# XiandaGuo/OpenStereo

Hardware: AMD Instinct MI355X
Metric: stereo-pairs/s at 540x960 D=192 (GwcNet fwd) (higher is better)
Workload: dtype f32 via f16x3 split-MFMA (hi/lo fp16 operands, f32 accumulate; HBM tensors f32); 1 GPU; GwcNet-gc inference, SceneFlow-shaped 540x960 padded to 544x960, D=192, G=40 + 12ch concat (BASELINE configs[1]); weights=deterministic synthetic (sharpened), random-init architecture, sub_batch_streams=3, parallelism=independent pairs x1, precision=f16x3, launch=hipGraph replay

## Files before the change

include/openstereo_amd.h:

```cpp
#ifndef OPENSTEREO_AMD_H
#define OPENSTEREO_AMD_H

#include <stddef.h>

#ifdef __cplusplus
extern "C" {
#endif

#define OSA_ABI_VERSION 17
#define OSA_META_FLOATS 128

enum { OSA_NCDHW = 0, OSA_NDHWC = 1 };
enum { OSA_ACT_NONE = 0, OSA_ACT_RELU = 1, OSA_ACT_LEAKY = 2, OSA_ACT_RELU6 = 3, OSA_ACT_SIGMOID = 4, OSA_ACT_TANH = 5 };
enum { OSA_GATE_RAW = 16 };
#define OSA_GATE_CHANNELS(n) ((int)((unsigned)(n) << 16))
enum { OSA_IN_SPLIT = 32, OSA_OUT_SPLIT = 64, OSA_RES_SPLIT = 128, OSA_REDIR_SPLIT = 256 };
enum { OSA_RES_AFTER_ACT = 512 };

int         osa_abi_version(void);
const char* osa_last_error(void);
const char* osa_target_arch(void);

int osa_build_volume_f32(const float* left_gwc, const float* right_gwc, int C, int num_groups,
                         const float* left_cat, const float* right_cat, int Cc,
                         float* vol, int layout, int vol_channels, int c_off,
                         int B, int H, int W, int maxdisp, int mask_left_concat,
                         float* vol_meta, void* stream);

int osa_build_volume_nhwc_f32(const float* left_gwc, const float* right_gwc, int C, int num_groups, int gwc_stride,
                              const float* left_cat, const float* right_cat, int Cc, int cat_stride,
                              float* vol, int vol_channels, int c_off,
                              int B, int H, int W, int maxdisp, int mask_left_concat, float* vol_meta, void* stream);
int osa_cat_fms_f32(const float* reference_fm, const float* target_fm, float* out, const int* disp_index,
                    int B, int C, int H, int W, int n_samples, void* stream);
int osa_pair_volume_f32(const float* left, const float* right, float* out,
                        int B, int C, int groups, int H, int W, int planes, int mode, void* stream);

int osa_corr_volume_f32(const float* left, const float* right, float* vol,
                        int B, int C, int H, int W, int maxdisp, void* stream);

int osa_ncdhw_to_ndhwc_f32(const float* x, float* y, int B, int C, long long S,
                           int yCs, int c_off, void* stream);
// ... 331 lines not shown
                            const float* mean3, const float* std3,
                            float* out, int layout, void* stream);

enum { OSA_IN_F16 = 32, OSA_OUT_F16 = 64, OSA_RES_F16 = 128 };
int osa_conv3d_pack_f16(const float* w_ref, float* w_packed, int Ci, int Co, int kd, int kh, int kw, void* stream);
int osa_deconv3d_pack_f16(const float* w_ref, float* w_packed, int Ci, int Co, int k, int pad, void* stream);
int osa_deconv2d_pack_f16(const float* w_ref, float* w_packed, int Ci, int Co, int k, int pad, void* stream);
int osa_conv3d_ndhwc_f16(const void* x, const float* w_packed, const float* scale, const float* shift, const void* residual, void* y,
                         int B, int Di, int Hi, int Wi, int Ci, int xCs, int Co, int yCs, int rCs, int kd, int kh, int kw, int stride,
                         int pad_d, int pad_h, int pad_w, int dil_d, int dil_h, int dil_w, const float* gate_logits, int gCs,
                         int act, float slope, void* stream);
int osa_deconv3d_ndhwc_f16(const void* x, const float* w_packed, const float* scale, const float* shift, const void* residual, void* y,
                           int B, int Di, int Hi, int Wi, int Ci, int xCs, int Co, int yCs, int rCs, int k, int pad, int opad,
                           const float* gate_logits, int gCs, int act, float slope, void* stream);
int osa_deconv2d_nhwc_f16(const void* x, const float* w_packed, const float* scale, const float* shift, const void* residual, void* y,
                          int B, int Hi, int Wi, int Ci, int xCs, int Co, int yCs, int rCs, int k, int pad, int opad,
                          const float* gate_logits, int gCs, int act, float slope, void* stream);

size_t osa_channel_sums_workspace_bytes(long long P, int C);
int osa_channel_sums(const void* dy, int dy_f16, int dy_cs, const void* x, int x_f16, int x_cs, const float* x_shift,
                     const float* dx_scale, void* dx, int dx_cs, long long P, int C,
                     float* out, float* workspace, size_t workspace_bytes, void* stream);
int osa_channel_sums_multi(const void* const* dys, int n_items, int dy_f16, int dy_cs, long long P, int C,
                           float* out, float* workspace, size_t workspace_bytes, void* stream);
int osa_channel_affine(const void* u, int u_f16, int u_cs, const void* v, int v_f16, int v_cs,
                       const float* a, const float* b, const float* c0, void* out, int out_cs,
                       long long P, int C, int relu, void* stream);

size_t osa_instnorm_workspace_floats(int B, long long HW, int C);
int osa_instnorm_nhwc_f32(const float* x, float* y, int B, long long HW, int C, int xCs, int yCs, float eps, int act, float slope,
                          float* workspace, float* y_meta, void* stream);

long long osa_conv3d_march_launches(void);

long long osa_conv3d_march_s2_launches(void);
int osa_conv_march_s2_segment_planes(int planes);

int osa_deconv_walk(int enable);
int osa_deconv_walk_segment_planes(int planes);
long long osa_deconv3d_walk_launches(void);

int osa_conv_b_ring_mask(int mask);
long long osa_conv_b_ring_launches(void);

int osa_volume_walk_step(int step);
long long osa_volume_walk_launches(void);

int osa_build_volume_nhwc_split_eligible(const float* left_cat, const float* right_cat, const float* vol, int C, int num_groups,
                                         int gwc_stride, int Cc, int cat_stride, int vol_channels, int c_off, int W, int maxdisp);
int osa_build_volume_nhwc_split_f16x3(const float* left_gwc, const float* right_gwc, int C, int num_groups, int gwc_stride,
                                      const float* left_cat, const float* right_cat, int Cc, int cat_stride,
                                      float* vol, int vol_channels, int c_off,
                                      int B, int H, int W, int maxdisp, int mask_left_concat,
                                      const float* gwc_meta, const float* cat_meta, float* vol_meta, void* stream);

#ifdef __cplusplus
}
#endif
#endif
```

openstereo_amd/_lib.py:

```python
from __future__ import annotations

import ctypes as C
import os
import threading

_HERE = os.path.dirname(os.path.abspath(__file__))
LIB_PATH = os.environ.get("OSA_LIB_PATH") or os.path.join(_HERE, "lib", "libopenstereo_amd.so")

_lock = threading.Lock()
_lib = None

c_fp = C.c_void_p
c_i = C.c_int
c_f = C.c_float
c_st = C.c_void_p
c_ll = C.c_longlong


class F16x3Ranges(C.Structure):
    _fields_ = [("x_meta", C.c_void_p), ("residual_meta", C.c_void_p), ("redir_meta", C.c_void_p),
                ("y_meta", C.c_void_p), ("bound_coef", C.c_void_p), ("redir_bound_coef", C.c_void_p), ("weight_scale", C.c_void_p)]


c_rng = C.POINTER(F16x3Ranges)
# ... 43 lines not shown
    **dict.fromkeys(("osa_deconv2d_nhwc_f32", "osa_deconv2d_nhwc_f16"), (c_i, [c_fp] * 6 + [c_i] * 11 + [c_fp, c_i, c_i, c_f, c_st])),
    "osa_deconv2d_nhwc_f16x3": (c_i, [c_fp] * 6 + [c_i] * 11 + [c_fp, c_i, c_i, c_f, c_f, c_rng, c_st]),
    "osa_dwconv2d_pack_f32": (c_i, [c_fp, c_fp, c_i, c_i, c_i, c_st]),
    "osa_dwconv2d_nhwc_f32": (c_i, [c_fp] * 6 + [c_i] * 15 + [c_fp, c_st]),
    "osa_dwconv2d_nhwc_f16io": (c_i, [c_fp, c_i, c_fp, c_fp, c_fp, c_fp, c_i] + [c_i] * 11 + [c_i, c_fp, c_st]),
    "osa_gru_combine_f32": (c_i, [c_fp, c_fp, c_fp, c_fp, c_ll, c_i, c_i, c_i, c_i, c_i, c_fp, c_st]),
    "osa_gru_gates_rz_fwd": (c_i, [c_ref, c_fp, c_fp, c_ref, c_ref, c_ref, c_ref, c_ref, c_ll, c_i, c_st]),
    "osa_gru_gates_rz_bwd": (c_i, [c_ref, c_fp, c_fp, c_ref, c_ref, c_ref, c_ref, c_ref, c_ref, c_ref, c_ll, c_i, c_st]),
    "osa_gru_gates_q_fwd": (c_i, [c_ref, c_ref, c_fp, c_ref, c_ref, c_ref, c_ll, c_i, c_st]),
    "osa_gru_gates_q_bwd": (c_i, [c_ref, c_ref, c_fp, c_ref, c_ref, c_ref, c_ref, c_ref, c_ref, c_ll, c_i, c_st]),
    "osa_disp_update_f32": (c_i, [c_fp, c_fp, c_i, c_fp, c_fp, c_i, c_ll, c_fp, c_fp, c_st]),
    "osa_conv3d_pack_ex_auto": (c_i, [c_fp, c_fp, c_i, c_i, c_i, c_i, c_i, c_i, c_i, c_fp, c_fp, c_st]),
    **dict.fromkeys(("osa_deconv3d_pack_f16x3_auto", "osa_deconv2d_pack_f16x3_auto"), (c_i, [c_fp, c_fp, c_i, c_i, c_i, c_i, c_fp, c_fp, c_st])),
    "osa_cat_fms_f32": (c_i, [c_fp, c_fp, c_fp, c_fp, c_i, c_i, c_i, c_i, c_i, c_st]),
    "osa_pool2x_nhwc_f32": (c_i, [c_fp, c_fp, c_i, c_i, c_i, c_i, c_i, c_i, c_fp, c_fp, c_st]),
    "osa_resize_bilinear_nhwc_f32": (c_i, [c_fp, c_fp, c_i, c_i, c_i, c_i, c_i, c_i, c_i, c_i, c_fp, c_fp, c_st]),
    "osa_context_upsample_logits_f32": (c_i, [c_fp, c_fp, c_i, C.POINTER(c_ll), c_fp, c_i, c_i, c_i, c_i, c_f, c_st]),
    "osa_context_upsample_logits_bwd_f32": (c_i, [c_fp, c_fp, c_i, C.POINTER(c_ll), c_fp, c_fp, c_fp, C.POINTER(c_ll), c_fp, c_i, c_i, c_i, c_i, c_f, c_st]),
    "osa_context_upsample_f32": (c_i, [c_fp, c_fp, c_fp, c_i, c_i, c_i, c_i, c_i, c_f, c_st]),
    "osa_geo_rows_f32": (c_i, [c_fp, c_fp, c_i, c_i, c_i, c_i, c_i, c_i, c_st]),
    "osa_avgpool_rows_f32": (c_i, [c_fp, c_fp, c_ll, c_i, c_st]),
    **dict.fromkeys(("osa_geo_lookup_f32", "osa_geo_lookup_bwd_acc_f32", "osa_geo_lookup_bwd_f32"), (c_i, _LEVELS + [c_fp, c_fp, c_fp, c_i, c_i, c_i, c_i, c_i, c_st])),
    "osa_geo_lookup_nhwc_f32": (c_i, _LEVELS + [c_fp, c_fp, c_fp, c_i, c_i, c_i, c_i, c_i, c_i, c_st]),
    **dict.fromkeys(("osa_geo_lookup_mr_f32", "osa_geo_lookup_mr_bwd_acc_f32"), (c_i, _LEVELS + [c_fp, c_i, c_fp, c_i, c_fp, c_fp, c_fp, c_fp, c_fp, c_fp, c_i, c_i, c_i, c_i, c_i, c_st])),
    "osa_geo_lookup_mr_nhwc_f32": (c_i, _LEVELS + [c_fp, c_i, c_fp, c_i, c_fp, c_fp, c_fp, c_fp, c_fp, c_fp, c_i, c_i, c_i, c_i, c_i, c_i, c_i, c_i, c_i, c_st]),
    "osa_preprocess_pair_f32": (c_i, [c_fp, c_fp, c_i, c_i, c_i, c_i, c_i, C.POINTER(c_f), C.POINTER(c_f), c_fp, c_i, c_st]),
    "osa_instnorm_workspace_floats": (C.c_size_t, [c_i, c_ll, c_i]),
    "osa_instnorm_nhwc_f32": (c_i, [c_fp, c_fp, c_i, c_ll, c_i, c_i, c_i, c_f, c_i, c_f, c_fp, c_fp, c_st]),
    "osa_conv3d_wgrad_ws_multi": (c_i, [c_i, c_fp, c_fp, c_i, c_fp] + [c_i] * 22 + [c_fp, c_fp, c_i, c_i, c_fp, C.c_size_t, c_st]),
    "osa_channel_sums_workspace_bytes": (C.c_size_t, [c_ll, c_i]),
    "osa_channel_affine": (c_i, [c_fp, c_i, c_i, c_fp, c_i, c_i, c_fp, c_fp, c_fp, c_fp, c_i, c_ll, c_i, c_i, c_st]),
    "osa_channel_sums_multi": (c_i, [c_fp, c_i, c_i, c_i, c_ll, c_i, c_fp, c_fp, C.c_size_t, c_st]),
    "osa_channel_sums": (c_i, [c_fp, c_i, c_i, c_fp, c_i, c_i, c_fp, c_fp, c_fp, c_i, c_ll, c_i, c_fp, c_fp, C.c_size_t, c_st]),
    **dict.fromkeys(("osa_conv3d_march_launches", "osa_conv3d_march_s2_launches", "osa_deconv3d_walk_launches", "osa_conv_b_ring_launches", "osa_volume_walk_launches"), (c_ll, [])),
    **dict.fromkeys(("osa_deconv_walk", "osa_deconv_walk_segment_planes", "osa_conv_march_s2_segment_planes", "osa_conv_b_ring_mask", "osa_volume_walk_step"), (c_i, [c_i])),
    "osa_build_volume_nhwc_split_eligible": (c_i, [c_fp, c_fp, c_fp, c_i, c_i, c_i, c_i, c_i, c_i, c_i, c_i, c_i]),
    "osa_build_volume_nhwc_split_f16x3": (c_i, [c_fp, c_fp, c_i, c_i, c_i, c_fp, c_fp, c_i, c_i, c_fp] + [c_i] * 7 + [c_fp, c_fp, c_fp, c_st]),
    "osa_upsample_softargmin_f32": (c_i, [c_fp, c_fp, c_i, c_i, c_i, c_i, c_i, c_i, c_i, c_i, c_st]),
    **dict.fromkeys(("osa_softargmin_var_f32", "osa_softmax_softargmin_var_bwd_f32"), (c_i, [c_fp, c_fp, c_fp, c_fp, c_i, c_i, c_i, c_i, c_st])),
    "osa_softargmin_var_bwd_f32": (c_i, [c_fp, c_fp, c_fp, c_fp, c_fp, c_fp, c_i, c_i, c_i, c_i, c_st]),
    "osa_upsample_softargmin_var_bwd_ws_f32": (c_i, [c_fp, c_fp, c_fp, c_fp, c_i, c_i, c_i, c_i, c_i, c_i, c_i, c_i, c_fp, C.c_size_t, c_st]),
    "osa_mr_volume_f32": (c_i, [c_fp] * 7 + [c_i] * 12 + [c_st]),
    "osa_mr_volume_bwd_ws_f32": (c_i, [c_fp] * 3 + [c_i] + [c_fp] * 8 + [c_i] * 11 + [c_fp, C.c_size_t, c_st]),
    **dict.fromkeys(("osa_mv2_block3d_packed_floats", "osa_mv2_block2d_packed_floats"), (C.c_size_t, [c_i] * 3)),
    **dict.fromkeys(("osa_mv2_block3d_pack_f32", "osa_mv2_block2d_pack_f32"), (c_i, [c_fp] * 10 + [c_i] * 3 + [c_st])),
    "osa_mv2_block3d_f32": (c_i, [c_fp] * 3 + [c_i] * 9 + [c_st]),
    **dict.fromkeys(("osa_mv2_block2d_f32", "osa_disparity_attention_f32"), (c_i, [c_fp] * 4 + [c_i] * 9 + [c_st])),
    "osa_disparity_attention_pack_f32": (c_i, [c_fp] * 8 + [c_i] * 4 + [c_st]),
    "osa_interlaced_volume_pack_f32": (c_i, [c_fp] * 13 + [c_i] * 4 + [c_st]),
    "osa_interlaced_volume_f32": (c_i, [c_fp] * 4 + [c_i] * 8 + [c_st]),
}


class EngineError(RuntimeError):
    pass


def load():
    global _lib
    if _lib is not None:
        return _lib
    with _lock:
        if _lib is not None:
            return _lib
        if not os.path.exists(LIB_PATH):
            raise EngineError(f"{LIB_PATH} is missing: build it with `python -m openstereo_amd.build` (hipcc, gfx950). There is no CPU fallback.")
        lib = C.CDLL(LIB_PATH)
        for name, (res, args) in SIGNATURES.items():
            fn = getattr(lib, name)
            fn.restype = res
            fn.argtypes = args
        if lib.osa_abi_version() != abi_version(lib):
            raise EngineError(f"ABI version mismatch: library reports {lib.osa_abi_version()}, include/openstereo_amd.h declares {abi_version(lib)}")
        if os.environ.get("OSA_B_RING_MASK"):
            lib.osa_conv_b_ring_mask(int(os.environ["OSA_B_RING_MASK"], 0))
        if os.environ.get("OSA_DECONV_WALK"):
            lib.osa_deconv_walk(int(os.environ["OSA_DECONV_WALK"], 0))
        if os.environ.get("OSA_VOL_WALK"):
            lib.osa_volume_walk_step(int(os.environ["OSA_VOL_WALK"]))
        _lib = lib
    return _lib


_abi = None


def abi_version(lib=None) -> int:
    global _abi
    if _abi is None:
        import re
        hdr = os.path.join(os.path.dirname(os.path.abspath(__file__)), "..", "include", "openstereo_amd.h")
        try:
            with open(hdr) as f:
                _abi = int(re.search(r"#define\s+OSA_ABI_VERSION\s+(\d+)", f.read()).group(1))
        except (OSError, AttributeError):
            h = lib if lib is not None else _lib
            if h is None:
                return -1
            _abi = int(h.osa_abi_version())
    return _abi


CALLS = {}


def call(name: str, *args):
    lib = load()
    CALLS[name] = CALLS.get(name, 0) + 1
    rc = getattr(lib, name)(*args)
    if rc != 0:
        msg = lib.osa_last_error()
        raise EngineError(f"{name} failed ({rc}): {msg.decode() if msg else '?'}")
# ... 2 lines not shown
```

openstereo_amd/csrc/conv_march.h:

```cpp
#pragma once
#include "conv_kernel.h"

namespace osa {

template <int NWV, int TW>
struct MarchGeo {
    static constexpr int MT = 2;
    static constexpr int RPT = 32 / TW;
    static constexpr int TH = NWV * MT * RPT;
    static constexpr int LH = TH + 2, LW = TW + 2;
    static constexpr int VQ = 5;
    static constexpr int ROWQ = (TW == 16) ? ((LW * VQ + 15) / 16 * 16) : LW * VQ;
    static constexpr int NPI = (LH * ROWQ + 63) / 64;
    static constexpr int PLANEQ = NPI * 64;
    static constexpr int NP = (NPI + NWV - 1) / NWV;
    static constexpr int NTHR = NWV * 64;
    static constexpr int BRING = 4;
    static constexpr int BSTEPQ = 6 * 64;
    static constexpr size_t lds_bytes() { return (size_t)2 * PLANEQ * 16 + (size_t)BRING * BSTEPQ * 16; }
    static_assert((size_t)NWV * 32 * 36 * 4 <= (size_t)PLANEQ * 16, "epilogue tiles must fit into one plane buffer");
    static_assert(NP <= 7, "one piece per wave and step, all of them forced home by the waits of steps 2..8");
};

template <int NWV, int TW, int OUTS, int INS>
__global__ __launch_bounds__(NWV * 64, 2) void conv_march_kernel(const ConvArgs p, const int dseg, const int nseg) {
    using G = MarchGeo<NWV, TW>;
    constexpr int MT = G::MT, TH = G::TH, ROWQ = G::ROWQ, VQ = G::VQ, PLANEQ = G::PLANEQ, NTHR = G::NTHR, NP = G::NP, NPI = G::NPI;
    extern __shared__ __attribute__((aligned(16))) float4 smem[];
    float4* const bring = smem + 2 * PLANEQ;

    const int tid = threadIdx.x, lane = tid & 63;
    const int wm = __builtin_amdgcn_readfirstlane(tid >> 6);
    const int col = lane & 31, hh = lane >> 5;

    unsigned bid = xcd_remap(blockIdx.x, gridDim.x);
    const int twi = bid % p.tilesW; bid /= p.tilesW;
    const int thi = bid % p.tilesH; bid /= p.tilesH;
    const int seg = bid % nseg;
    const int b = (int)(bid / nseg);
    const int d0 = seg * dseg, d1 = (d0 + dseg < p.Di) ? d0 + dseg : p.Di;
    const int a0h = thi * TH, a0w = twi * TW;
    const int g0h = a0h - 1, g0w = a0w - 1;

    float s_in = 1.f, s_res_inv = 1.f, s_out = 1.f;
    if (p.in_meta) s_in = INS ? p.in_meta[1] : pow2_scale(amax_read(p.in_meta));
    if (p.res && p.res_meta && (p.act & OSA_RES_SPLIT)) s_res_inv = 1.0f / p.res_meta[1];
    if (OUTS && p.coef && p.in_meta) {
        float bound = p.coef[0] * amax_read(p.in_meta) + p.coef[1];
        if (p.res && p.res_meta) bound += amax_read(p.res_meta);
        s_out = pow2_scale(bound * 1.0625f);
    }
    if (OUTS && p.out_meta && blockIdx.x == 0 && tid == 0) p.out_meta[1] = s_out;
    const float osc = (p.wscale_dev ? p.wscale_dev[1] : p.oscale) * (1.0f / s_in);
    float am = 0.f;
    unsigned amax_seen = 0u;
    if (p.out_meta) amax_seen = amax_peek(p.out_meta);

    int abase[MT];
#pragma unroll
    for (int m = 0; m < MT; ++m) {
        const int q = (wm * MT + m) * 32 + col;
        abase[m] = (q / TW) * ROWQ + (q % TW) * VQ + hh;
    }

    f32x16 acc[3][MT];
#pragma unroll
    for (int s = 0; s < 3; ++s)
#pragma unroll
        for (int m = 0; m < MT; ++m)
#pragma unroll
            for (int r = 0; r < 16; ++r) acc[s][m][r] = 0.f;

    const int bstep = 2 * p.CoP;
    const int tstep = 2 * bstep;
// ... 121 lines not shown
                            r = mul4(r, s_res_inv);
                        }
                        float o[4] = {fmaf(a.x, sc[h2].x, sh[h2].x) + r.x, fmaf(a.y, sc[h2].y, sh[h2].y) + r.y,
                                      fmaf(a.z, sc[h2].z, sh[h2].z) + r.z, fmaf(a.w, sc[h2].w, sh[h2].w) + r.w};
#pragma unroll
                        for (int e = 0; e < 4; ++e) o[e] = (o[e] < 0.f) ? (act_relu ? 0.f : o[e] * act_ns) : o[e];
                        if (ok) am = fmaxf(am, fmaxf(fmaxf(fabsf(o[0]), fabsf(o[1])), fmaxf(fabsf(o[2]), fabsf(o[3]))));
                        split_f16(make_float4(o[0] * s_out, o[1] * s_out, o[2] * s_out, o[3] * s_out), hq[h2], lq[h2]);
                    }
                    if (ok) {
                        float* ys = yb + vox * p.yCs + soff;
                        store16(ys, make_uint4(hq[0].x, hq[0].y, hq[1].x, hq[1].y));
                        store16(ys + 8, make_uint4(lq[0].x, lq[0].y, lq[1].x, lq[1].y));
                    }
                }
            }
        }
    };


    const int pf = (d0 - 1 > 0) ? d0 - 1 : 0, pl = (d1 < p.Di - 1) ? d1 : p.Di - 1;
    const int npass = (pl - pf + 1) * nch;
    if constexpr (INS) {
#pragma unroll
        for (int i = 0; i < NP; ++i) dma_piece(i, 0, pf, 0);
    }
    dma_b(0, 0, 0); dma_b(1, 0, 1); dma_b(2, 0, 2);

    int pd = pf, c = 0;
    for (int q = 0; q < npass; ++q) {
        const int cn = (c + 1 < nch) ? c + 1 : 0;
        const int pdn = (q + 1 < npass) ? ((c + 1 < nch) ? pd : pd + 1) : -1;
        const int sb = q & 3, cur = q & 1;
        if constexpr (!INS) {
            __syncthreads();
            stage_brick<NTHR, PREC_F16X3, 1, 4>(p, smem + cur * PLANEQ, PLANEQ, b, c * CC, pd, g0h, g0w, tid, s_in);
        }
        if (!INS || q == 0) asm volatile("s_waitcnt vmcnt(0)" ::: "memory");
        __syncthreads();
        int ab[MT];
#pragma unroll
        for (int m = 0; m < MT; ++m) ab[m] = abase[m] + cur * PLANEQ;
        int bq[4];
#pragma unroll
        for (int k = 0; k < 4; ++k) bq[k] = (((sb + k) & 3) * 6) * 64 + lane;
        float4 A[2][MT][2], B[3][2];
        auto load_a = [&](float4 (&An)[MT][2], const int khw) {
            const int off = (khw / 3) * ROWQ + (khw % 3) * VQ;
#pragma unroll
            for (int m = 0; m < MT; ++m) { An[m][0] = smem[ab[m] + off]; An[m][1] = smem[ab[m] + off + 2]; }
        };
        auto load_b = [&](float4 (&Bn)[2], const int u) {
            const int kd = u % 3;
            Bn[0] = bring[bq[(u / 3) & 3] + (kd * 2) * 64]; Bn[1] = bring[bq[(u / 3) & 3] + (kd * 2 + 1) * 64];
        };
        load_b(B[0], 0);
        load_b(B[1], 1);
        load_a(A[0], 0);
#pragma unroll
        for (int s = 0; s < 9; ++s) {
            if (s > 0) { __builtin_amdgcn_s_barrier(); asm volatile("" ::: "memory"); }
            if (s + 3 < 9) dma_b((sb + s + 3) & 3, c, s + 3);
            else dma_b((sb + s + 3) & 3, cn, s + 3 - 9);
            if (s < NP) dma_piece(s, cur ^ 1, pdn, cn);
            if (s + 1 < 9) load_a(A[(s + 1) & 1], s + 1);
#pragma unroll
            for (int kd = 0; kd < 3; ++kd) {
                const int u = s * 3 + kd;
                if (u + 2 < 27) load_b(B[(u + 2) % 3], u + 2);
                __builtin_amdgcn_sched_barrier(0);
#pragma unroll
                for (int term = 0; term < 3; ++term)
#pragma unroll
                    for (int m = 0; m < MT; ++m) {
                        const f16x8 a = __builtin_bit_cast(f16x8, A[s & 1][m][term == 1 ? 1 : 0]);
                        const f16x8 w = __builtin_bit_cast(f16x8, B[u % 3][term == 0 ? 1 : 0]);
                        acc[2 - kd][m] = __builtin_amdgcn_mfma_f32_32x32x16_f16(a, w, acc[2 - kd][m], 0, 0, 0);
                    }
                __builtin_amdgcn_sched_barrier(0);
            }
            constexpr int PCS = INS ? 1 : 0;
            wait_vmcnt(NI + ((s < NP) ? PCS : 0) + ((s >= 1 && s - 1 < NP) ? PCS : 0));
        }
        if (c + 1 == nch) {
            const bool v2 = (pd - 1 >= d0) && (pd - 1 < d1);
            if (v2) {
                __syncthreads();
                epilogue(pd - 1, reinterpret_cast<float*>(smem + cur * PLANEQ) + wm * (32 * 36));
            }
#pragma unroll
            for (int m = 0; m < MT; ++m) {
                acc[0][m] = acc[1][m]; acc[1][m] = acc[2][m];
#pragma unroll
                for (int r = 0; r < 16; ++r) acc[2][m][r] = 0.f;
            }
            if (q + 1 == npass && pd + 1 == d1 && pd + 1 >= p.Di) {
                __syncthreads();
                epilogue(pd, reinterpret_cast<float*>(smem + cur * PLANEQ) + wm * (32 * 36));
            }
            ++pd; c = 0;
        } else ++c;
    }
    asm volatile("s_waitcnt vmcnt(0)" ::: "memory");
    if (p.out_meta) {
        __syncthreads();
        publish_amax(p.out_meta, am, amax_seen, reinterpret_cast<float*>(smem));
    }
}

}
```

openstereo_amd/csrc/conv_march.hip:

```cpp
#include "conv_march.h"
#include "conv_march_s2.h"
#include "conv_deconv_walk.h"

namespace osa {

static long long g_march_launches = 0;
long long march_launches() { return g_march_launches; }

struct MarchCfg { int nwv, tw, th; size_t lds; void (*fn[2][2])(const ConvArgs, int, int); };
#define OSA_MARCH_CFG(NWV, TW) { NWV, TW, MarchGeo<NWV, TW>::TH, MarchGeo<NWV, TW>::lds_bytes(),                      \
                                 { { conv_march_kernel<NWV, TW, 0, 0>, conv_march_kernel<NWV, TW, 0, 1> },            \
                                   { conv_march_kernel<NWV, TW, 1, 0>, conv_march_kernel<NWV, TW, 1, 1> } } }
static const MarchCfg g_march_cfgs[] = {
    OSA_MARCH_CFG(4, 16),
    OSA_MARCH_CFG(4, 32),
};

int launch_conv_march(ConvArgs& a, hipStream_t st, const char* what) {
    if (!exp_int("OSA_MARCH", 1)) return 0;
    if (a.T != 27 || a.Co != 32 || a.CoP != 32 || a.Di < 3 || a.gate || a.rx) return 0;
    if (a.Ci % 16 != 0) return 0;
    const int actk = a.act & 15;
    if (actk > OSA_ACT_LEAKY || (a.act & (OSA_GATE_RAW | OSA_RES_AFTER_ACT)) || ((unsigned)a.act >> 16)) return 0;
    if ((a.yCs & 3) || ((size_t)a.y & 15) || (a.res && ((a.rCs & 3) || ((size_t)a.res & 15)))) return 0;
    if ((long long)a.Do * a.Ho * a.Wo * (a.yCs > a.rCs ? a.yCs : a.rCs) >= (1ll << 31)) return 0;
    if ((long long)a.Di * a.Hi * a.Wi * a.xCs >= (1ll << 31)) return 0;
    if (a.act & OSA_IN_SPLIT) OSA_REQUIRE(a.Ci % 16 == 0, "%s: split input needs Ci %% 16 == 0 (got %d)", what, a.Ci);
    if (a.act & OSA_OUT_SPLIT) {
        OSA_REQUIRE(a.yCs % 16 == 0, "%s: split output needs yCs %% 16 == 0", what);
        if (a.res) OSA_REQUIRE(a.act & OSA_RES_SPLIT, "%s: a split output takes a split residual", what);
    }
    if ((a.act & OSA_RES_SPLIT) && a.res) OSA_REQUIRE(a.rCs % 16 == 0, "%s: split residual needs rCs %% 16 == 0", what);
    int gi = exp_int("OSA_MARCH_GEO", -1);
    if (gi < 0 || gi > 1) {
        long long best = -1;
        for (int i = 0; i < 2; ++i) {
            const MarchCfg& g = g_march_cfgs[i];
            const long long area = (long long)cdiv(a.Ho, g.th) * g.th * cdiv(a.Wo, g.tw) * g.tw;
            if (best < 0 || area < best) { best = area; gi = i; }
        }
    }
    const MarchCfg& g = g_march_cfgs[gi];
    a.tilesD = 1; a.tilesH = cdiv(a.Ho, g.th); a.tilesW = cdiv(a.Wo, g.tw);
    a.dmin = a.hmin = a.wmin = -1;
    a.LD = 1; a.LH = g.th + 2; a.LW = g.tw + 2;
    a.VQ = 5;
    a.RowQ = (g.tw == 16) ? ((a.LW * 5 + 15) / 16 * 16) : a.LW * 5;
    a.PlaneQ = a.LH * a.RowQ;
    a.magicW = (unsigned)((0x100000000ull + a.LW - 1) / a.LW);
    a.magicH = (unsigned)((0x100000000ull + a.LH - 1) / a.LH);
    a.magicHW = (unsigned)((0x100000000ull + (unsigned long long)a.LH * a.LW - 1) / ((unsigned long long)a.LH * a.LW));
    a.cps = 1; a.dma = 0; a.dbg = exp_int("OSA_DBG", 0);
    const long long cols = (long long)a.B * a.tilesH * a.tilesW;
    int per_cu = (int)((160 * 1024) / g.lds);
    if (per_cu > 8 / g.nwv) per_cu = 8 / g.nwv;
    const long long slots = (long long)per_cu * 256;
    int nseg = 1;
    {
        double best = 1e30;
        for (int n = 1; n <= 16 && n * 2 <= a.Di; ++n) {
            const int ds = cdiv(a.Di, n), ns = cdiv(a.Di, ds);
            if (ns != n) continue;
            const double cost = (double)((cols * ns + slots - 1) / slots) * (ds + (ns > 1 ? 2.0 : 0.0));
            if (cost < best - 1e-9) { best = cost; nseg = ns; }
        }
        const int o = exp_int("OSA_MARCH_NSEG", 0);
        if (o > 0 && o * 2 <= a.Di) nseg = o;
    }
    const int dseg = cdiv(a.Di, nseg);
    nseg = cdiv(a.Di, dseg);
    OSA_REQUIRE(cols * nseg < (1ll << 31), "%s: grid too large", what);
    void (*fn)(const ConvArgs, int, int) = g.fn[(a.act & OSA_OUT_SPLIT) ? 1 : 0][(a.act & OSA_IN_SPLIT) ? 1 : 0];
    static bool attr_set[2][2][2];
    bool& done = attr_set[gi][(a.act & OSA_OUT_SPLIT) ? 1 : 0][(a.act & OSA_IN_SPLIT) ? 1 : 0];
    if (!done && g.lds > 64 * 1024) { (void)hipFuncSetAttribute((const void*)fn, hipFuncAttributeMaxDynamicSharedMemorySize, (int)g.lds); }
    done = true;
    hipLaunchKernelGGL(fn, dim3((unsigned)(cols * nseg)), dim3(g.nwv * 64), g.lds, st, a, dseg, nseg);
    OSA_LAUNCH_CHECK(what);
    ++g_march_launches;
    return 1;
}

static long long g_march_s2_launches = 0;
long long march_s2_launches() { return g_march_s2_launches; }

static int g_march_s2_planes = 0;
int march_s2_planes_set(int planes) { const int prev = g_march_s2_planes; g_march_s2_planes = planes > 0 ? planes : 0; return prev; }

int launch_conv_march_s2(ConvArgs& a, hipStream_t st, const char* what) {
    if (a.T != 27 || a.Co != 64 || a.CoP != 64 || a.Di < 2 || a.gate || a.rx || a.res) return 0;
    if (a.Ci % 16 != 0 || a.xCs % 16 != 0) return 0;
    if (!(a.act & OSA_IN_SPLIT) || !(a.act & OSA_OUT_SPLIT)) return 0;
    const int actk = a.act & 15;
    if (actk > OSA_ACT_LEAKY || (a.act & (OSA_GATE_RAW | OSA_RES_AFTER_ACT)) || ((unsigned)a.act >> 16)) return 0;
    if ((a.yCs % 16) || ((size_t)a.y & 15) || ((size_t)a.x & 15)) return 0;
    if ((long long)a.Do * a.Ho * a.Wo * a.yCs >= (1ll << 31)) return 0;
    if ((long long)a.Hi * a.Wi * a.xCs >= (1ll << 29)) return 0;
    using G = MarchS2Geo;
    a.tilesD = 1; a.tilesH = cdiv(a.Ho, G::TH); a.tilesW = cdiv(a.Wo, G::TW);
    const long long cols = (long long)a.B * a.tilesH * a.tilesW;
    const long long slots = 256;
    int nseg = 1;
    {
        double best = 1e30;
        for (int n = 1; n <= a.Do; ++n) {
            const int os = cdiv(a.Do, n), ns = cdiv(a.Do, os);
            if (ns != n) continue;
            const double cost = (double)((cols * ns + slots - 1) / slots) * (3.0 * os + (ns > 1 ? 1.0 : 0.0) + 1.5);
            if (cost < best - 1e-9) { best = cost; nseg = ns; }
        }
    }
    int oseg = cdiv(a.Do, nseg);
// ... 44 lines not shown
        }
    }
    int oseg = cdiv(a.Do, nseg);
    if (g_deconv_walk_planes > 0) oseg = g_deconv_walk_planes < a.Do ? g_deconv_walk_planes : a.Do;
    nseg = cdiv(a.Do, oseg);
    OSA_REQUIRE(cols * nseg < (1ll << 31), "%s: grid too large", what);
    OSA_REQUIRE(hipFuncSetAttribute((const void*)conv_deconv_walk_kernel<WN, RCH>, hipFuncAttributeMaxDynamicSharedMemorySize, (int)G::lds_bytes()) == hipSuccess,
                "%s: %d bytes of LDS per workgroup refused", what, (int)G::lds_bytes());
    hipLaunchKernelGGL((conv_deconv_walk_kernel<WN, RCH>), dim3((unsigned)(cols * nseg)), dim3(G::NWV * 64), G::lds_bytes(), st, a, oseg, nseg);
    OSA_LAUNCH_CHECK(what);
    return 1;
}

int launch_conv_deconv_walk(ConvArgs& a, hipStream_t st, const char* what) {
    if (a.T != 27 || a.Do != 2 * a.Di || a.Ho != 2 * a.Hi || a.Wo != 2 * a.Wi) return 0;
    if (!a.rx || a.res || a.gate) return 0;
    const int cls = (a.Co == 32 && a.rCi == 32) ? 0 : ((a.Co == 64 && a.rCi == 64) ? 1 : -1);
    if (cls < 0 || a.CoP != a.Co || !((g_deconv_walk >> cls) & 1)) return 0;
    if (!(a.act & OSA_IN_SPLIT) || !(a.act & OSA_OUT_SPLIT) || !(a.act & OSA_REDIR_SPLIT)) return 0;
    const int actk = a.act & 15;
    if (actk > OSA_ACT_LEAKY || (a.act & (OSA_GATE_RAW | OSA_RES_AFTER_ACT)) || ((unsigned)a.act >> 16)) return 0;
    if (a.Ci % 16 != 0 || a.xCs % 16 != 0 || a.yCs % 16 != 0 || a.rxCs % 16 != 0) return 0;
    if (((size_t)a.x & 15) || ((size_t)a.y & 15) || ((size_t)a.rx & 15)) return 0;
    if ((long long)a.Do * a.Ho * a.Wo * (a.yCs > a.rxCs ? a.yCs : a.rxCs) >= (1ll << 31)) return 0;
    if ((long long)a.Hi * a.Wi * a.xCs >= (1ll << 29)) return 0;
    const int r = cls == 0 ? launch_conv_deconv_walk_t<1, 2>(a, st, what) : launch_conv_deconv_walk_t<2, 4>(a, st, what);
    if (r == 1) ++g_deconv_walk_launches;
    return r;
}

}

extern "C" long long osa_conv3d_march_launches(void) { return osa::march_launches(); }
extern "C" long long osa_conv3d_march_s2_launches(void) { return osa::march_s2_launches(); }
extern "C" int osa_conv_march_s2_segment_planes(int planes) { return osa::march_s2_planes_set(planes); }
extern "C" long long osa_deconv3d_walk_launches(void) { return osa::deconv_walk_launches(); }
extern "C" int osa_deconv_walk(int enable) { return osa::deconv_walk_set(enable); }
extern "C" int osa_deconv_walk_segment_planes(int planes) { return osa::deconv_walk_planes_set(planes); }
```

Baseline: 196.4 stereo-pairs/s.

## Add mixed-geometry march tiling, boundary kd-skip, and dedicated f32 staging

The 3D conv march kernel now has a planner that can tile the bulk of the image with 16-wide tiles and the leftover rows with 32-wide tiles in a single mixed launch, which cuts padded tile area at H=136/68-like shapes. With plan mode 3 on by default, it also skips MFMA work for kd taps that fall outside the depth segment. That lets segment-count selection drop the halo penalty and use fewer segments when the grid already fills the GPU. A dedicated f32 staging routine with 4-way unrolled loads replaces the generic stage_brick. The costs are a larger kernel body with a two-way branch, which may raise register pressure, and more complex planning logic.

```diff
diff --git a/include/openstereo_amd.h b/include/openstereo_amd.h
--- a/include/openstereo_amd.h
+++ b/include/openstereo_amd.h
@@ -7,7 +7,7 @@
 extern "C" {
 #endif
 
-#define OSA_ABI_VERSION 17
+#define OSA_ABI_VERSION 18
 #define OSA_META_FLOATS 128
 
 enum { OSA_NCDHW = 0, OSA_NDHWC = 1 };
@@ -405,6 +405,10 @@
                           float* workspace, float* y_meta, void* stream);
 
 long long osa_conv3d_march_launches(void);
+long long osa_conv3d_march_mixed_launches(void);
+int osa_conv_march_plan(int mode);
+int osa_conv_march_segments(int n);
+int osa_conv_march_tiling(int B, int Di, int Ho, int Wo, int* out);
 
 long long osa_conv3d_march_s2_launches(void);
 int osa_conv_march_s2_segment_planes(int planes);
diff --git a/openstereo_amd/_lib.py b/openstereo_amd/_lib.py
--- a/openstereo_amd/_lib.py
+++ b/openstereo_amd/_lib.py
@@ -99,8 +99,8 @@
     "osa_channel_affine": (c_i, [c_fp, c_i, c_i, c_fp, c_i, c_i, c_fp, c_fp, c_fp, c_fp, c_i, c_ll, c_i, c_i, c_st]),
     "osa_channel_sums_multi": (c_i, [c_fp, c_i, c_i, c_i, c_ll, c_i, c_fp, c_fp, C.c_size_t, c_st]),
     "osa_channel_sums": (c_i, [c_fp, c_i, c_i, c_fp, c_i, c_i, c_fp, c_fp, c_fp, c_i, c_ll, c_i, c_fp, c_fp, C.c_size_t, c_st]),
-    **dict.fromkeys(("osa_conv3d_march_launches", "osa_conv3d_march_s2_launches", "osa_deconv3d_walk_launches", "osa_conv_b_ring_launches", "osa_volume_walk_launches"), (c_ll, [])),
-    **dict.fromkeys(("osa_deconv_walk", "osa_deconv_walk_segment_planes", "osa_conv_march_s2_segment_planes", "osa_conv_b_ring_mask", "osa_volume_walk_step"), (c_i, [c_i])),
+    **dict.fromkeys(("osa_conv3d_march_launches", "osa_conv3d_march_mixed_launches", "osa_conv3d_march_s2_launches", "osa_deconv3d_walk_launches", "osa_conv_b_ring_launches", "osa_volume_walk_launches"), (c_ll, [])),
+    **dict.fromkeys(("osa_deconv_walk", "osa_deconv_walk_segment_planes", "osa_conv_march_s2_segment_planes", "osa_conv_b_ring_mask", "osa_volume_walk_step", "osa_conv_march_plan", "osa_conv_march_segments"), (c_i, [c_i])), "osa_conv_march_tiling": (c_i, [c_i] * 4 + [C.POINTER(c_i)]),
     "osa_build_volume_nhwc_split_eligible": (c_i, [c_fp, c_fp, c_fp, c_i, c_i, c_i, c_i, c_i, c_i, c_i, c_i, c_i]),
     "osa_build_volume_nhwc_split_f16x3": (c_i, [c_fp, c_fp, c_i, c_i, c_i, c_fp, c_fp, c_i, c_i, c_fp] + [c_i] * 7 + [c_fp, c_fp, c_fp, c_st]),
     "osa_upsample_softargmin_f32": (c_i, [c_fp, c_fp, c_i, c_i, c_i, c_i, c_i, c_i, c_i, c_i, c_st]),
@@ -139,12 +139,12 @@
             fn.argtypes = args
         if lib.osa_abi_version() != abi_version(lib):
             raise EngineError(f"ABI version mismatch: library reports {lib.osa_abi_version()}, include/openstereo_amd.h declares {abi_version(lib)}")
-        if os.environ.get("OSA_B_RING_MASK"):
-            lib.osa_conv_b_ring_mask(int(os.environ["OSA_B_RING_MASK"], 0))
-        if os.environ.get("OSA_DECONV_WALK"):
-            lib.osa_deconv_walk(int(os.environ["OSA_DECONV_WALK"], 0))
-        if os.environ.get("OSA_VOL_WALK"):
-            lib.osa_volume_walk_step(int(os.environ["OSA_VOL_WALK"]))
+        for env, setter in (("OSA_B_RING_MASK", lib.osa_conv_b_ring_mask),
+                            ("OSA_DECONV_WALK", lib.osa_deconv_walk),
+                            ("OSA_MARCH_PLAN", lib.osa_conv_march_plan),
+                            ("OSA_VOL_WALK", lib.osa_volume_walk_step)):
+            if os.environ.get(env):
+                setter(int(os.environ[env], 0))
         _lib = lib
     return _lib
 
diff --git a/openstereo_amd/csrc/conv_march.h b/openstereo_amd/csrc/conv_march.h
--- a/openstereo_amd/csrc/conv_march.h
+++ b/openstereo_amd/csrc/conv_march.h
@@ -22,10 +22,49 @@
     static_assert(NP <= 7, "one piece per wave and step, all of them forced home by the waits of steps 2..8");
 };
 
+struct MarchTile { int b, seg, a0h, a0w; };
+
+struct MarchMix { int n0, n1, tilesW0, h1; };
+
+template <class G>
+__device__ __forceinline__ void march_stage_f32(const ConvArgs& p, float4* dst, const int b, const int c0, const int pd,
+                                                const int g0h, const int g0w, const int tid, const float s_in) {
+    constexpr int U = 4, NTHR = G::NTHR, total = G::LH * G::LW * (CC / 4);
+    static_assert(NTHR % 4 == 0, "channel quad of an item must not depend on u");
+    const float* xb = p.x + ((size_t)b * p.Di + pd) * p.Hi * p.Wi * p.xCs + c0;
+    const int c4 = tid & 3;
+    uint2* const s2 = reinterpret_cast<uint2*>(dst);
+    for (int base = tid; base < total; base += NTHR * U) {
+        float4 v[U];
+        int lo[U];
+#pragma unroll
+        for (int u = 0; u < U; ++u) {
+            const int it = base + u * NTHR;
+            lo[u] = -1;
+            v[u] = make_float4(0.f, 0.f, 0.f, 0.f);
+            if (it < total) {
+                const int vx = it >> 2, lh = vx / G::LW, lw = vx - lh * G::LW;
+                const int gh = g0h + lh, gw = g0w + lw;
+                lo[u] = lh * G::ROWQ + lw * G::VQ;
+                if ((unsigned)gh < (unsigned)p.Hi && (unsigned)gw < (unsigned)p.Wi && c0 + c4 * 4 < p.Ci)
+                    v[u] = *reinterpret_cast<const float4*>(xb + (gh * p.Wi + gw) * p.xCs + c4 * 4);
+            }
+        }
+#pragma unroll
+        for (int u = 0; u < U; ++u)
+            if (lo[u] >= 0) {
+                uint2 h2, l2;
+                split_f16(mul4(v[u], s_in), h2, l2);
+                s2[lo[u] * 2 + c4] = h2;
+                s2[lo[u] * 2 + 4 + c4] = l2;
+            }
+    }
+}
+
 template <int NWV, int TW, int OUTS, int INS>
-__global__ __launch_bounds__(NWV * 64, 2) void conv_march_kernel(const ConvArgs p, const int dseg, const int nseg) {
+__device__ __forceinline__ void conv_march_body(const ConvArgs& p, const int dseg, const int kdskip, const MarchTile t) {
     using G = MarchGeo<NWV, TW>;
-    constexpr int MT = G::MT, TH = G::TH, ROWQ = G::ROWQ, VQ = G::VQ, PLANEQ = G::PLANEQ, NTHR = G::NTHR, NP = G::NP, NPI = G::NPI;
+    constexpr int MT = G::MT, ROWQ = G::ROWQ, VQ = G::VQ, PLANEQ = G::PLANEQ, NP = G::NP, NPI = G::NPI;
     extern __shared__ __attribute__((aligned(16))) float4 smem[];
     float4* const bring = smem + 2 * PLANEQ;
 
@@ -33,13 +72,9 @@
     const int wm = __builtin_amdgcn_readfirstlane(tid >> 6);
     const int col = lane & 31, hh = lane >> 5;
 
-    unsigned bid = xcd_remap(blockIdx.x, gridDim.x);
-    const int twi = bid % p.tilesW; bid /= p.tilesW;
-    const int thi = bid % p.tilesH; bid /= p.tilesH;
-    const int seg = bid % nseg;
-    const int b = (int)(bid / nseg);
-    const int d0 = seg * dseg, d1 = (d0 + dseg < p.Di) ? d0 + dseg : p.Di;
-    const int a0h = thi * TH, a0w = twi * TW;
+    const int b = t.b;
+    const int d0 = t.seg * dseg, d1 = (d0 + dseg < p.Di) ? d0 + dseg : p.Di;
+    const int a0h = t.a0h, a0w = t.a0w;
     const int g0h = a0h - 1, g0w = a0w - 1;
 
     float s_in = 1.f, s_res_inv = 1.f, s_out = 1.f;
@@ -227,9 +262,11 @@
         const int cn = (c + 1 < nch) ? c + 1 : 0;
         const int pdn = (q + 1 < npass) ? ((c + 1 < nch) ? pd : pd + 1) : -1;
         const int sb = q & 3, cur = q & 1;
+        unsigned live = 7u;
+        if (kdskip) live = (pd + 1 < d1 ? 1u : 0u) | ((pd >= d0 && pd < d1) ? 2u : 0u) | (pd - 1 >= d0 ? 4u : 0u);
         if constexpr (!INS) {
             __syncthreads();
-            stage_brick<NTHR, PREC_F16X3, 1, 4>(p, smem + cur * PLANEQ, PLANEQ, b, c * CC, pd, g0h, g0w, tid, s_in);
+            march_stage_f32<G>(p, smem + cur * PLANEQ, b, c * CC, pd, g0h, g0w, tid, s_in);
         }
         if (!INS || q == 0) asm volatile("s_waitcnt vmcnt(0)" ::: "memory");
         __syncthreads();
@@ -264,14 +301,16 @@
                 const int u = s * 3 + kd;
                 if (u + 2 < 27) load_b(B[(u + 2) % 3], u + 2);
                 __builtin_amdgcn_sched_barrier(0);
-#pragma unroll
-                for (int term = 0; term < 3; ++term)
-#pragma unroll
-                    for (int m = 0; m < MT; ++m) {
-                        const f16x8 a = __builtin_bit_cast(f16x8, A[s & 1][m][term == 1 ? 1 : 0]);
-                        const f16x8 w = __builtin_bit_cast(f16x8, B[u % 3][term == 0 ? 1 : 0]);
-                        acc[2 - kd][m] = __builtin_amdgcn_mfma_f32_32x32x16_f16(a, w, acc[2 - kd][m], 0, 0, 0);
-                    }
+                if (live & (1u << kd)) {
+#pragma unroll
+                    for (int term = 0; term < 3; ++term)
+#pragma unroll
+                        for (int m = 0; m < MT; ++m) {
+                            const f16x8 a = __builtin_bit_cast(f16x8, A[s & 1][m][term == 1 ? 1 : 0]);
+                            const f16x8 w = __builtin_bit_cast(f16x8, B[u % 3][term == 0 ? 1 : 0]);
+                            acc[2 - kd][m] = __builtin_amdgcn_mfma_f32_32x32x16_f16(a, w, acc[2 - kd][m], 0, 0, 0);
+                        }
+                }
                 __builtin_amdgcn_sched_barrier(0);
             }
             constexpr int PCS = INS ? 1 : 0;
@@ -303,4 +342,33 @@
     }
 }
 
-}
+template <int NWV, int TW, int OUTS, int INS>
+__global__ __launch_bounds__(NWV * 64, 2) void conv_march_kernel(const ConvArgs p, const int dseg, const int nseg, const int kdskip) {
+    unsigned bid = xcd_remap(blockIdx.x, gridDim.x);
+    const int twi = bid % p.tilesW; bid /= p.tilesW;
+    const int thi = bid % p.tilesH; bid /= p.tilesH;
+    MarchTile t;
+    t.seg = bid % nseg; t.b = (int)(bid / nseg);
+    t.a0h = thi * MarchGeo<NWV, TW>::TH; t.a0w = twi * TW;
+    conv_march_body<NWV, TW, OUTS, INS>(p, dseg, kdskip, t);
+}
+
+template <int OUTS, int INS>
+__global__ __launch_bounds__(256, 2) void conv_march_mixed_kernel(const ConvArgs p, const int dseg, const int nseg, const int kdskip, const MarchMix mx) {
+    static_assert(MarchGeo<4, 16>::lds_bytes() == MarchGeo<4, 32>::lds_bytes(), "one LDS size for both bodies");
+    unsigned bid = xcd_remap(blockIdx.x, gridDim.x);
+    const unsigned cpi = (unsigned)(mx.n0 + mx.n1);
+    const int ti = (int)(bid % cpi); bid /= cpi;
+    MarchTile t;
+    t.seg = bid % nseg; t.b = (int)(bid / nseg);
+    if (ti < mx.n0) {
+        const int thi = ti / mx.tilesW0;
+        t.a0h = thi * MarchGeo<4, 16>::TH; t.a0w = (ti - thi * mx.tilesW0) * 16;
+        conv_march_body<4, 16, OUTS, INS>(p, dseg, kdskip, t);
+    } else {
+        t.a0h = mx.h1; t.a0w = (ti - mx.n0) * 32;
+        conv_march_body<4, 32, OUTS, INS>(p, dseg, kdskip, t);
+    }
+}
+
+}
diff --git a/openstereo_amd/csrc/conv_march.hip b/openstereo_amd/csrc/conv_march.hip
--- a/openstereo_amd/csrc/conv_march.hip
+++ b/openstereo_amd/csrc/conv_march.hip
@@ -4,10 +4,16 @@
 
 namespace osa {
 
-static long long g_march_launches = 0;
+static long long g_march_launches = 0, g_march_mixed_launches = 0;
 long long march_launches() { return g_march_launches; }
-
-struct MarchCfg { int nwv, tw, th; size_t lds; void (*fn[2][2])(const ConvArgs, int, int); };
+long long march_mixed_launches() { return g_march_mixed_launches; }
+
+static int g_march_plan = 3;
+int march_plan_set(int mode) { const int prev = g_march_plan; g_march_plan = mode & 7; return prev; }
+static int g_march_segments = 0;
+int march_segments_set(int n) { const int prev = g_march_segments; g_march_segments = n > 0 ? n : 0; return prev; }
+
+struct MarchCfg { int nwv, tw, th; size_t lds; void (*fn[2][2])(const ConvArgs, int, int, int); };
 #define OSA_MARCH_CFG(NWV, TW) { NWV, TW, MarchGeo<NWV, TW>::TH, MarchGeo<NWV, TW>::lds_bytes(),                      \
                                  { { conv_march_kernel<NWV, TW, 0, 0>, conv_march_kernel<NWV, TW, 0, 1> },            \
                                    { conv_march_kernel<NWV, TW, 1, 0>, conv_march_kernel<NWV, TW, 1, 1> } } }
@@ -15,6 +21,76 @@
     OSA_MARCH_CFG(4, 16),
     OSA_MARCH_CFG(4, 32),
 };
+static void (*const g_march_mixed_fn[2][2])(const ConvArgs, int, int, int, const MarchMix) = {
+    { conv_march_mixed_kernel<0, 0>, conv_march_mixed_kernel<0, 1> }, { conv_march_mixed_kernel<1, 0>, conv_march_mixed_kernel<1, 1> } };
+
+struct MarchRegion { int gi, h0, w0, h1, w1, tilesH, tilesW; };
+struct MarchPlan { int nreg; MarchRegion r[2]; long long area; int cols_img, nseg, dseg; };
+
+static MarchRegion march_region(int gi, int h0, int w0, int h1, int w1) {
+    const MarchCfg& g = g_march_cfgs[gi];
+    return MarchRegion{gi, h0, w0, h1, w1, cdiv(h1 - h0, g.th), cdiv(w1 - w0, g.tw)};
+}
+static long long march_area(const MarchRegion& r) {
+    return (long long)r.tilesH * g_march_cfgs[r.gi].th * r.tilesW * g_march_cfgs[r.gi].tw;
+}
+
+static constexpr double MARCH_CUT_FULL = 2.0, MARCH_CUT_SKIP = 2.0 / 3.0;
+
+static MarchPlan march_plan(int B, int Di, int Ho, int Wo, int mode, int geo, int force_nseg) {
+    MarchPlan pl{};
+    if (geo < 0 || geo > 1) {
+        long long best = -1;
+        for (int i = 0; i < 2; ++i) {
+            const long long area = march_area(march_region(i, 0, 0, Ho, Wo));
+            if (best < 0 || area < best) { best = area; geo = i; }
+        }
+        pl.nreg = 1; pl.r[0] = march_region(geo, 0, 0, Ho, Wo); pl.area = best;
+        if (mode & 1) {
+            const int hm = Ho - Ho % 16;
+            if (hm > 0 && Ho % 16 > 0 && Ho % 16 <= 8) {
+                const MarchRegion r0 = march_region(0, 0, 0, hm, Wo), r1 = march_region(1, hm, 0, Ho, Wo);
+                const long long area = march_area(r0) + march_area(r1);
+                if (area < pl.area) { pl.nreg = 2; pl.r[0] = r0; pl.r[1] = r1; pl.area = area; }
+            }
+        }
+    } else {
+        pl.nreg = 1; pl.r[0] = march_region(geo, 0, 0, Ho, Wo); pl.area = march_area(pl.r[0]);
+    }
+    pl.cols_img = 0;
+    for (int i = 0; i < pl.nreg; ++i) pl.cols_img += pl.r[i].tilesH * pl.r[i].tilesW;
+    const long long cols = (long long)B * pl.cols_img;
+    const MarchCfg& g = g_march_cfgs[pl.r[0].gi];
+    int per_cu = (int)((160 * 1024) / g.lds);
+    if (per_cu > 8 / g.nwv) per_cu = 8 / g.nwv;
+    const long long slots = (long long)per_cu * 256;
+    const double cut = (mode & 2) ? MARCH_CUT_SKIP : MARCH_CUT_FULL;
+    int nseg = 1;
+    if ((mode & 4) || !(mode & 2) || cols > slots) {
+        double best = 1e30;
+        for (int n = 1; n <= 16 && n * 2 <= Di; ++n) {
+            const int ds = cdiv(Di, n), ns = cdiv(Di, ds);
+            if (ns != n) continue;
+            const double cost = (double)((cols * ns + slots - 1) / slots) * (ds + (ns > 1 ? cut : 0.0));
+            if (cost < best - 1e-9) { best = cost; nseg = ns; }
+        }
+    }
+    if (force_nseg > 0 && force_nseg * 2 <= Di) nseg = force_nseg;
+    pl.dseg = cdiv(Di, nseg);
+    pl.nseg = cdiv(Di, pl.dseg);
+    return pl;
+}
+
+int march_tiling(int B, int Di, int Ho, int Wo, int* out) {
+    const MarchPlan pl = march_plan(B, Di, Ho, Wo, g_march_plan, -1, g_march_segments);
+    out[0] = pl.nreg; out[1] = pl.cols_img; out[2] = pl.nseg; out[3] = pl.dseg; out[4] = (int)pl.area;
+    for (int i = 0; i < 2; ++i) {
+        int* o = out + 5 + 5 * i;
+        if (i < pl.nreg) { o[0] = pl.r[i].h0; o[1] = pl.r[i].w0; o[2] = pl.r[i].h1; o[3] = pl.r[i].w1; o[4] = g_march_cfgs[pl.r[i].gi].tw; }
+        else o[0] = o[1] = o[2] = o[3] = o[4] = 0;
+    }
+    return 0;
+}
 
 int launch_conv_march(ConvArgs& a, hipStream_t st, const char* what) {
     if (!exp_int("OSA_MARCH", 1)) return 0;
@@ -31,53 +107,34 @@
         if (a.res) OSA_REQUIRE(a.act & OSA_RES_SPLIT, "%s: a split output takes a split residual", what);
     }
     if ((a.act & OSA_RES_SPLIT) && a.res) OSA_REQUIRE(a.rCs % 16 == 0, "%s: split residual needs rCs %% 16 == 0", what);
-    int gi = exp_int("OSA_MARCH_GEO", -1);
-    if (gi < 0 || gi > 1) {
-        long long best = -1;
-        for (int i = 0; i < 2; ++i) {
-            const MarchCfg& g = g_march_cfgs[i];
-            const long long area = (long long)cdiv(a.Ho, g.th) * g.th * cdiv(a.Wo, g.tw) * g.tw;
-            if (best < 0 || area < best) { best = area; gi = i; }
-        }
-    }
+    int force = exp_int("OSA_MARCH_NSEG", 0);
+    if (force <= 0) force = g_march_segments;
+    const MarchPlan pl = march_plan(a.B, a.Di, a.Ho, a.Wo, g_march_plan, exp_int("OSA_MARCH_GEO", -1), force);
+    const int kdskip = (g_march_plan >> 1) & 1, os = (a.act & OSA_OUT_SPLIT) ? 1 : 0, is = (a.act & OSA_IN_SPLIT) ? 1 : 0;
+    const int gi = pl.r[0].gi;
     const MarchCfg& g = g_march_cfgs[gi];
-    a.tilesD = 1; a.tilesH = cdiv(a.Ho, g.th); a.tilesW = cdiv(a.Wo, g.tw);
-    a.dmin = a.hmin = a.wmin = -1;
-    a.LD = 1; a.LH = g.th + 2; a.LW = g.tw + 2;
-    a.VQ = 5;
-    a.RowQ = (g.tw == 16) ? ((a.LW * 5 + 15) / 16 * 16) : a.LW * 5;
-    a.PlaneQ = a.LH * a.RowQ;
-    a.magicW = (unsigned)((0x100000000ull + a.LW - 1) / a.LW);
-    a.magicH = (unsigned)((0x100000000ull + a.LH - 1) / a.LH);
-    a.magicHW = (unsigned)((0x100000000ull + (unsigned long long)a.LH * a.LW - 1) / ((unsigned long long)a.LH * a.LW));
+    a.tilesD = 1; a.tilesH = pl.r[0].tilesH; a.tilesW = pl.r[0].tilesW;
     a.cps = 1; a.dma = 0; a.dbg = exp_int("OSA_DBG", 0);
-    const long long cols = (long long)a.B * a.tilesH * a.tilesW;
-    int per_cu = (int)((160 * 1024) / g.lds);
-    if (per_cu > 8 / g.nwv) per_cu = 8 / g.nwv;
-    const long long slots = (long long)per_cu * 256;
-    int nseg = 1;
-    {
-        double best = 1e30;
-        for (int n = 1; n <= 16 && n * 2 <= a.Di; ++n) {
-            const int ds = cdiv(a.Di, n), ns = cdiv(a.Di, ds);
-            if (ns != n) continue;
-            const double cost = (double)((cols * ns + slots - 1) / slots) * (ds + (ns > 1 ? 2.0 : 0.0));
-            if (cost < best - 1e-9) { best = cost; nseg = ns; }
-        }
-        const int o = exp_int("OSA_MARCH_NSEG", 0);
-        if (o > 0 && o * 2 <= a.Di) nseg = o;
-    }
-    const int dseg = cdiv(a.Di, nseg);
-    nseg = cdiv(a.Di, dseg);
-    OSA_REQUIRE(cols * nseg < (1ll << 31), "%s: grid too large", what);
-    void (*fn)(const ConvArgs, int, int) = g.fn[(a.act & OSA_OUT_SPLIT) ? 1 : 0][(a.act & OSA_IN_SPLIT) ? 1 : 0];
-    static bool attr_set[2][2][2];
-    bool& done = attr_set[gi][(a.act & OSA_OUT_SPLIT) ? 1 : 0][(a.act & OSA_IN_SPLIT) ? 1 : 0];
-    if (!done && g.lds > 64 * 1024) { (void)hipFuncSetAttribute((const void*)fn, hipFuncAttributeMaxDynamicSharedMemorySize, (int)g.lds); }
-    done = true;
-    hipLaunchKernelGGL(fn, dim3((unsigned)(cols * nseg)), dim3(g.nwv * 64), g.lds, st, a, dseg, nseg);
+    const long long cols = (long long)a.B * pl.cols_img;
+    OSA_REQUIRE(cols * pl.nseg < (1ll << 31), "%s: grid too large", what);
+    static bool attr_set[3][2][2];
+    bool& done = attr_set[pl.nreg == 2 ? 2 : gi][os][is];
+    if (pl.nreg == 1) {
+        void (*fn)(const ConvArgs, int, int, int) = g.fn[os][is];
+        if (!done && g.lds > 64 * 1024) { (void)hipFuncSetAttribute((const void*)fn, hipFuncAttributeMaxDynamicSharedMemorySize, (int)g.lds); }
+        done = true;
+        hipLaunchKernelGGL(fn, dim3((unsigned)(cols * pl.nseg)), dim3(g.nwv * 64), g.lds, st, a, pl.dseg, pl.nseg, kdskip);
+    } else {
+        void (*fn)(const ConvArgs, int, int, int, const MarchMix) = g_march_mixed_fn[os][is];
+        if (!done && g.lds > 64 * 1024) { (void)hipFuncSetAttribute((const void*)fn, hipFuncAttributeMaxDynamicSharedMemorySize, (int)g.lds); }
+        done = true;
+        const MarchRegion &r0 = pl.r[0], &r1 = pl.r[1];
+        const MarchMix mx{r0.tilesH * r0.tilesW, r1.tilesW, r0.tilesW, r1.h0};
+        hipLaunchKernelGGL(fn, dim3((unsigned)(cols * pl.nseg)), dim3(256), g.lds, st, a, pl.dseg, pl.nseg, kdskip, mx);
+    }
     OSA_LAUNCH_CHECK(what);
     ++g_march_launches;
+    if (pl.nreg == 2) ++g_march_mixed_launches;
     return 1;
 }
 
@@ -188,6 +245,16 @@
 }
 
 extern "C" long long osa_conv3d_march_launches(void) { return osa::march_launches(); }
+extern "C" long long osa_conv3d_march_mixed_launches(void) { return osa::march_mixed_launches(); }
+extern "C" int osa_conv_march_plan(int mode) { return osa::march_plan_set(mode); }
+extern "C" int osa_conv_march_segments(int n) { return osa::march_segments_set(n); }
+extern "C" int osa_conv_march_tiling(int B, int Di, int Ho, int Wo, int* out) {
+    if (B < 1 || Di < 3 || Ho < 1 || Wo < 1 || !out || (long long)(Ho + 16) * (Wo + 32) >= (1ll << 31)) {
+        osa::set_error("osa_conv_march_tiling: needs B >= 1, Di >= 3, Ho, Wo >= 1 and a 15-int result array");
+        return -1;
+    }
+    return osa::march_tiling(B, Di, Ho, Wo, out);
+}
 extern "C" long long osa_conv3d_march_s2_launches(void) { return osa::march_s2_launches(); }
 extern "C" int osa_conv_march_s2_segment_planes(int planes) { return osa::march_s2_planes_set(planes); }
 extern "C" long long osa_deconv3d_walk_launches(void) { return osa::deconv_walk_launches(); }
```

New measurement: 198.2 stereo-pairs/s (median of 6 runs). No clear change (+0.9%).
